# jy2k/Kubeflow-v2-distributed-pytorch

Measured on AMD Instinct MI355X. Metric: samples/sec (whole node) task.py DDP at 1/2/4/8 MI355X; scaling efficiency, higher is better.
Workload: dtype bf16; 1 GPU; model=resnet50, global_batch=256, image_size=224, batch_per_gpu=256, parallelism=dp1, impl=mipipe, optimizer=SGD(lr=0.1,momentum=0.9,wd=1e-4), hip_graph=True, deterministic=False, force_reduce=False, comm_dtype=fp32, native_reducer=False

## Files before the change

### csrc/bindings.cpp

```cpp
#include <torch/extension.h>

#include <unordered_map>

#include "bind/common.hpp"

using namespace mipipe_bind;

namespace {

void check_conv_buf_bytes(const mipipe::ConvShape& s, bool f32, const char* what) {
  if (f32) return;
  const int64_t lim = (1ll << 31) - (1ll << 24);
  TORCH_CHECK((int64_t)s.N * s.H * s.W * s.Ci * 2 < lim && (int64_t)s.N * s.Ho * s.Wo * s.Co * 2 < lim,
              "bf16 ", what, " tensors beyond 2 GiB are not supported");
}

mipipe::ConvShape make_conv_shape(int64_t N, int64_t H, int64_t W, int64_t Ci, int64_t Co, int KH,
                                  int KW, int stride, int pad, int stride_w, int pad_w, bool f32) {
  mipipe::ConvShape s;
  s.N = (int)N; s.H = (int)H; s.W = (int)W; s.Ci = (int)Ci;
  s.Co = (int)Co; s.KH = KH; s.KW = KW; s.stride = stride; s.pad = pad;
  s.stride_w = stride_w > 0 ? stride_w : 0;
  s.pad_w = pad_w >= 0 ? pad_w : -1;
  s.f32 = f32;
// ... 277 lines not shown
      mipipe::conv_fwd_infer(x.data_ptr(), w.data_ptr(), ys.data_ptr(), s, stream(), scp, shp, rp,
                             relu, c, wsp(ws));
    });
  }
  Tensor ws = split_ws(mipipe::conv_fwd_split_ws_elems(s, cfg), x);
  mipipe::conv_fwd_infer(x.data_ptr(), w.data_ptr(), y.data_ptr(), s, stream(), scp, shp, rp, relu,
                         cfg, wsp(ws));
  return y;
}

Tensor conv_dgrad(Tensor dy, Tensor w, std::vector<int64_t> x_shape, int stride, int pad,
                  optional<Tensor> addend, optional<Tensor> bn_y, optional<Tensor> bn_mean,
                  optional<Tensor> bn_invstd, optional<Tensor> bn_scale, optional<Tensor> bn_bias,
                  optional<Tensor> bn_rep, optional<Tensor> bn_z, int pad_w, int cfg,
                  optional<Tensor> bn_mask, optional<Tensor> bn_y2, optional<Tensor> bn_mean2,
                  optional<Tensor> bn_invstd2, optional<Tensor> wflip_pre) {
  check_act(dy, "dy");
  check_same(w, dy, "w");
  c10::DeviceGuard g(dy.device());
  TORCH_CHECK(x_shape.size() == 4, "x_shape must be [N,H,W,Ci]");
  const auto s = make_conv_shape(x_shape[0], x_shape[1], x_shape[2], x_shape[3], w.size(0),
                                 (int)w.size(1), (int)w.size(2), stride, pad, 0, pad_w, is_f32(dy));
  TORCH_CHECK(w.size(3) == s.Ci, "weight/input channel mismatch");
  const int pw = pad_w >= 0 ? pad_w : pad;
  TORCH_CHECK(dy.size(0) == s.N && dy.size(1) == s.Ho && dy.size(2) == s.Wo && dy.size(3) == s.Co,
              "dy shape does not match the convolution");
  TORCH_CHECK(s.Ci % 8 == 0 && s.Co % 8 == 0, "conv dgrad needs Ci, Co % 8 == 0");
  TORCH_CHECK(dy.numel() < (1ll << 31), "conv dgrad dy too large for 32-bit gather offsets");
  check_conv_buf_bytes(s, s.f32, "conv dgrad");
  TORCH_CHECK(s.pad < s.KH && pw < s.KW, "conv dgrad expects padding < kernel size");
  auto dx = torch::empty({s.N, s.H, s.W, s.Ci}, dy.options());
// ... 6 lines not shown
    if (wflip_pre.has_value() && mipipe::dgrad_preflip_ok(s)) {
      check_same(*wflip_pre, w, "wflip_pre");
      TORCH_CHECK(wflip_pre->numel() == w.numel() && wflip_pre->is_contiguous(),
                  "wflip_pre must match w's size");
      wfp = wflip_pre->data_ptr();
      preflipped = true;
    } else {
      wflip = torch::empty({(int64_t)s.Ci * s.KH * s.KW * s.Co}, w.options());
      wfp = wflip.data_ptr();
    }
  }
  mipipe::DgradFusion fz;
  bool any = false;
  if (addend.has_value()) {
    check_same(*addend, dy, "addend");
    TORCH_CHECK(addend->sizes() == dx.sizes(), "addend must match dx");
    fz.addend = addend->data_ptr();
    any = true;
  }
  if (bn_rep.has_value()) {
    TORCH_CHECK(bn_y.has_value() && bn_mean.has_value() && bn_invstd.has_value() &&
                bn_scale.has_value() && bn_bias.has_value(), "BN fusion needs y/mean/invstd/scale/bias");
    check_same(*bn_y, dy, "bn_y");
    TORCH_CHECK(bn_y->sizes() == dx.sizes(), "bn_y must match dx");
    check_vec(*bn_mean, s.Ci, "bn_mean");
    check_vec(*bn_invstd, s.Ci, "bn_invstd");
    check_vec(*bn_scale, s.Ci, "bn_scale");
    check_vec(*bn_bias, s.Ci, "bn_bias");
    check_f32(*bn_rep, "bn_rep");
    TORCH_CHECK(bn_rep->numel() == 3ll * mipipe::kStatReplicas * s.Ci, "bn_rep must be [3,R,Ci]");
    for (const Tensor* t : {&*bn_mean, &*bn_invstd, &*bn_scale, &*bn_bias})
      TORCH_CHECK(reinterpret_cast<uintptr_t>(t->data_ptr()) % 16 == 0,
                  "BN fusion vectors must be 16-byte aligned (the epilogue reads them as float4)");
// ... 1572 lines not shown
  m.attr("BN_ROW_ITERS") = mipipe::kBnRowIters;
  m.attr("DET_CHUNK_ROWS") = mipipe::kDetChunkRows;
  m.def("bn_bwd_reduce_blocks", [](int64_t M, int64_t C) {
    TORCH_CHECK(M >= 0 && C >= 8 && C % 8 == 0, "bn_bwd_reduce_blocks: M >= 0, C % 8 == 0");
    return mipipe::bn_bwd_reduce_blocks((long)M, (int)C);
  });
  m.def("bn_apply_u", []() { return mipipe::bn_apply_u(); });
  m.def("conv_dgrad", &conv_dgrad, py::arg("dy"), py::arg("w"), py::arg("x_shape"),
        py::arg("stride"), py::arg("pad"), py::arg("addend") = py::none(),
        py::arg("bn_y") = py::none(), py::arg("bn_mean") = py::none(),
        py::arg("bn_invstd") = py::none(), py::arg("bn_scale") = py::none(),
        py::arg("bn_bias") = py::none(), py::arg("bn_rep") = py::none(),
        py::arg("bn_z") = py::none(), py::arg("pad_w") = -1, py::arg("cfg") = -1,
        py::arg("bn_mask") = py::none(), py::arg("bn_y2") = py::none(),
        py::arg("bn_mean2") = py::none(), py::arg("bn_invstd2") = py::none(),
        py::arg("wflip_pre") = py::none());
  m.def("dgrad_preflip_ok", [](std::vector<int64_t> x_shape, std::vector<int64_t> w_shape,
                               int stride, int pad) {
    return mipipe::dgrad_preflip_ok(make_conv_shape(x_shape[0], x_shape[1], x_shape[2], x_shape[3],
                                                    w_shape[0], (int)w_shape[1], (int)w_shape[2],
                                                    stride, pad, 0, -1, false));
  });
  m.def("bn_bwd_collect", &bn_bwd_collect, py::arg("rep"), py::arg("C"),
        py::arg("dgamma") = py::none(), py::arg("dbeta") = py::none());
  m.def("conv_wgrad", &conv_wgrad, py::arg("dy"), py::arg("x"), py::arg("kh"), py::arg("kw"),
        py::arg("stride"), py::arg("pad"), py::arg("out") = py::none(), py::arg("stride_w") = 0,
        py::arg("pad_w") = -1, py::arg("cfg") = -1, py::arg("col_rep") = py::none(),
        py::arg("col_out") = py::none(), py::arg("col_dgamma") = py::none(),
        py::arg("col_dbeta") = py::none(), py::arg("col_two") = false,
        py::arg("col_dgamma2") = py::none(), py::arg("col_dbeta2") = py::none(),
        py::arg("in_scale") = py::none(), py::arg("in_bias") = py::none());
// ... 149 lines not shown
```

### csrc/kernels/conv_common.hpp

```cpp
#pragma once
#include "epilogue.hpp"
#include "gemm_pp.hpp"
#include "launchers.hpp"

namespace mipipe {
namespace gk {

static __device__ __attribute__((aligned(64))) uint4 g_conv_zero[8];

template <int BM_, int BN_, int NS_, int WM_, int WN_, bool PP_ = false>
struct Tile {
  static constexpr int BM = BM_, BN = BN_, NS = NS_, WM = WM_, WN = WN_;
  static constexpr int NW = WM * WN;
  static constexpr int THREADS = 64 * NW;
  static constexpr bool PP = PP_;
};

typedef Tile<128, 128, 2, 2, 2> T0;
typedef Tile<128, 128, 1, 2, 2> T1;
typedef Tile<128, 64, 2, 2, 2> T2;
typedef Tile<256, 128, 2, 4, 2> T3;
typedef Tile<256, 128, 3, 4, 2> T4;
typedef Tile<128, 256, 2, 2, 4> T5;
typedef Tile<256, 256, 2, 4, 2> T6;
// ... 109 lines not shown
  if (std::is_same<T, float>::value && f32_stages<C::BM, C::BN>() == 2) return 1;
  return C::NW == 8 ? (C::BM * C::BN <= 128 * 128 ? 2 : 1)
                    : ((C::NS == 1 && !std::is_same<T, float>::value) ? 3 : 2);
}

template <class T, class C, bool SPLIT>
constexpr int conv_fwd_lds_bytes() {
  return SPLIT && lds_bytes_f32out<T, C>() > lds_bytes_out<T, C>() ? lds_bytes_f32out<T, C>()
                                                                   : lds_bytes_out<T, C>();
}
template <class T, class C, bool BNIN>
constexpr int bnin_lds_bytes() {
  return BNIN ? main_lds_bytes<T, C>() + kBnInMaxK * 8 : 0;
}
template <class C, bool DENSE, bool ALIGNED, class T, bool DGRAD_EPI = false, bool SPLIT = false,
          bool BNIN = false>
__global__ __launch_bounds__(C::THREADS, (conv_occ<T, C>())) void conv_fwd_kernel(
    const T* __restrict__ x, const T* __restrict__ w, ConvGeom g, uint32_t M,
    uint32_t tilesN, EpiParams e) {
  constexpr int BM = C::BM, BN = C::BN;
  static_assert(!BNIN || (DENSE && !C::PP && !SPLIT && !DGRAD_EPI), "folded-BN forward variant");
  typedef typename std::conditional<
      BNIN, PolKCDenseBN<T>,
      typename std::conditional<DENSE, PolKCDense<T>, PolKCIm2col<ALIGNED, T>>::type>::type PA;
  constexpr int kLds = conv_fwd_lds_bytes<T, C, SPLIT>() > bnin_lds_bytes<T, C, BNIN>()
                           ? conv_fwd_lds_bytes<T, C, SPLIT>()
                           : bnin_lds_bytes<T, C, BNIN>();
  __shared__ __attribute__((aligned(16))) char smem[kLds];
  const int wave = __builtin_amdgcn_readfirstlane(threadIdx.x >> 6);
  const int lane = threadIdx.x & 63;
  uint32_t ntile = gridDim.x;
  if constexpr (!DGRAD_EPI) {
    if (e.fl_wt != nullptr) {
      if (blockIdx.x >= e.fl_tiles) {
        if (SPLIT && blockIdx.y != 0) return;
        flip_block<T, C::THREADS>(e, blockIdx.x - e.fl_tiles, smem);
// ... 23 lines not shown
    else a.init(x, g, M, origin, wave, lane, g_conv_zero);
    if constexpr (BNIN) a.tab = bn_tab;
  };
  auto ib = [&](auto& b, uint32_t origin) { b.init(w, K, e.N, K, origin, wave, lane, g_conv_zero); };
  f32x4 acc[BM / C::WM / 16][BN / C::WN / 16];
  run_main_loop<T, C, PA, PolKCDense<T>>(smem, ia, ib, m0, n0, kt0, kt1, acc, wave, lane);
  if constexpr (SPLIT) {
    EpiParams ws{};
    ws.C = e.split_ws;
    ws.ldc = e.N;
    ws.M = M;
    ws.N = e.N;
    ws.det_rows = 1;
    epilogue_f32<BM, BN, true, C::WM, C::WN, C::PP>(smem, acc, ws, m0, n0, wave, lane);
  } else {
    epilogue_out<BM, BN, DGRAD_EPI, T, C::WM, C::WN, false, C::PP>(smem, acc, e, m0, n0, 0, wave,
                                                                   lane);
  }
}

template <class T, class C>
constexpr int finish_lds_bytes() {
  constexpr int a = kEpiLdsBytes<C::BM, C::BN, T, C::WM>();
  constexpr int b = 16 * (C::THREADS + 8) * 4;
  return a > b ? a : b;
}
template <class C, class T, bool FUSE>
__global__ __launch_bounds__(C::THREADS) void conv_splitk_finish_kernel(
    const float* __restrict__ ws, int S, uint32_t tilesN, EpiParams e) {
  constexpr int BM = C::BM, BN = C::BN, WM = C::WM, WN = C::WN;
  constexpr int MT = BM / WM / 16, NT = BN / WN / 16;
  __shared__ __attribute__((aligned(16))) char smem[finish_lds_bytes<T, C>()];
  const int wave = __builtin_amdgcn_readfirstlane(threadIdx.x >> 6);
  const int lane = threadIdx.x & 63;
  const uint32_t tm = blockIdx.x / tilesN, tn = blockIdx.x % tilesN;
  const uint32_t m0 = tm * BM, n0 = tn * BN;
  const int wr = wave / WN, wc = wave % WN;
  typedef AccMap<BM, BN, WM, WN, false> Map;
  const uint32_t lr = lane & 15, lc = (lane >> 4) * 4;
  const long slice = (long)e.M * e.N;
  long off[MT][NT];
#pragma unroll
// ... 10 lines not shown
#pragma unroll
    for (int j = 0; j < NT; ++j) {
      const float4 v = *reinterpret_cast<const float4*>(ws + off[i][j]);
      acc[i][j] = f32x4{v.x, v.y, v.z, v.w};
    }
  for (int s = 1; s < S; ++s) {
    const float* wsl = ws + s * slice;
#pragma unroll
    for (int i = 0; i < MT; ++i)
#pragma unroll
      for (int j = 0; j < NT; ++j) {
        const float4 v = *reinterpret_cast<const float4*>(wsl + off[i][j]);
        acc[i][j] += f32x4{v.x, v.y, v.z, v.w};
      }
  }
  epilogue_out<BM, BN, FUSE, T, WM, WN, false, false>(smem, acc, e, m0, n0, 0, wave, lane);
}

template <class C, bool DENSE, bool ALIGNED, class T, bool TWO = false>
__global__ __launch_bounds__(C::THREADS, (conv_occ<T, C>())) void conv_dgrad_kernel(
    const T* __restrict__ dy, const T* __restrict__ w, int Ho, int Wo, int Co, int taps,
    FastDiv fCo, DgradClass cls, uint32_t M, uint32_t tilesN, EpiParams e) {
  constexpr int BM = C::BM, BN = C::BN;
  typedef typename std::conditional<DENSE, PolKCDense<T>, PolKCDgrad<ALIGNED, T>>::type PA;
  typedef typename std::conditional<DENSE, PolMCDense<T>, PolMCDgradW<ALIGNED, T>>::type PB;
  __shared__ __attribute__((aligned(16))) char smem[lds_bytes_out<T, C>()];
  const int wave = __builtin_amdgcn_readfirstlane(threadIdx.x >> 6);
  const int lane = threadIdx.x & 63;
  const uint32_t id = xcd_remap(blockIdx.x, gridDim.x);
  const uint32_t tm = id / tilesN, tn = id % tilesN;
  const uint32_t m0 = tm * BM, n0 = tn * BN;
  const uint32_t Ci = e.N;
  const uint32_t K = (uint32_t)(cls.ntaps * Co);
  const int nk = (int)((K + BK - 1) / BK);
  auto ia = [&](auto& a, uint32_t origin) {
    if constexpr (DENSE) a.init(dy, Co, M, K, origin, wave, lane, g_conv_zero);
    else a.init(dy, Ho, Wo, Co, fCo, cls, M, origin, wave, lane, g_conv_zero);
  };
  auto ib = [&](auto& b, uint32_t origin) {
    if constexpr (DENSE) b.init(w, Ci, Ci, K, origin, wave, lane, g_conv_zero);
    else b.init(w, (uint32_t)Co, (uint32_t)taps, Ci, fCo, cls, origin, wave, lane, g_conv_zero);
  };
  f32x4 acc[BM / C::WM / 16][BN / C::WN / 16];
  run_main_loop<T, C, PA, PB>(smem, ia, ib, m0, n0, 0, nk, acc, wave, lane);
  epilogue_out<BM, BN, true, T, C::WM, C::WN, TWO, C::PP>(smem, acc, e, m0, n0, 0, wave, lane);
}

template <class C, bool DENSE, class T, bool ATOMIC = true, bool BNIN = false>
__global__ __launch_bounds__(C::THREADS, (conv_occ<T, C>())) void conv_wgrad_kernel(
    const T* __restrict__ dy, const T* __restrict__ x, ConvGeom g, uint32_t tilesN,
    int kt_per_split, EpiParams e) {
  constexpr int BM = C::BM, BN = C::BN;
  static_assert(!BNIN || (DENSE && !C::PP), "folded-BN weight-grad variant");
  typedef typename std::conditional<
      BNIN, PolMCDenseBN<T>,
      typename std::conditional<DENSE, PolMCDense<T>, PolMCIm2colT<T>>::type>::type PB;
  __shared__ __attribute__((aligned(16))) char smem[lds_bytes_f32out<T, C>()];
  const int wave = __builtin_amdgcn_readfirstlane(threadIdx.x >> 6);
  const int lane = threadIdx.x & 63;
  const SplitPos pos = splitk_pos(e.xcd_splits);
// ... 81 lines not shown
```

### csrc/kernels/conv_dgrad.hip

```cpp
#include "conv_common.hpp"

namespace mipipe {
using namespace gk;

int default_dgrad_cfg(const ConvShape& s, long K_class) {
  const bool dense = is_dense(s);
  const bool ns1 = !s.f32 && (dense ? s.Co <= g_ns1_max_k
                                    : (s.Co % BK == 0 && K_class <= g_ns1_max_k_gather));
  if (s.Ci <= 64) return 2;
  return ns1 ? 1 : 0;
}

template <class F>
static void for_each_class(const ConvShape& s, F&& f) {
  const int S = s.stride;
  const int PW = s.pad_w >= 0 ? s.pad_w : s.pad;
  for (int ph = 0; ph < S; ++ph) {
    for (int pw = 0; pw < S; ++pw) {
      DgradClass c{};
      c.ph = ph; c.pw = pw;
      c.Hc = (s.H - ph + S - 1) / S;
      c.Wc = (s.W - pw + S - 1) / S;
      if (c.Hc <= 0 || c.Wc <= 0) continue;
      c.S = S; c.KW = s.KW;
// ... 134 lines not shown
      e.nt = ((g_nt_store >> 1) & 1) &&
             (long)s.N * s.H * s.W * s.Ci * (s.f32 ? 4 : 2) > g_nt_min_bytes;
      e.ntl = (g_nt_store >> 8) & 1;
      if (fz != nullptr) {
        e.addend = fz->addend;
        e.bnr_y = fz->bn_y;
        e.bnr_mean = fz->bn_mean; e.bnr_invstd = fz->bn_invstd;
        e.bnr_scale = fz->bn_scale; e.bnr_bias = fz->bn_bias; e.bnr_rep = fz->bn_rep; e.st_R = g_stat_rows;
        e.bnr_z = fz->bn_z;
        e.bnr_mask = fz->bn_mask;
        e.bnr_y2 = fz->bn_y2;
        e.bnr_mean2 = fz->bn_mean2;
        e.bnr_invstd2 = fz->bn_invstd2;
        e.det_rows = fz->det_rows;
        e.det_row0 = row0;
      }
      if (S > 1) {
        e.rm_s = S; e.rm_ph = c.ph; e.rm_pw = c.pw; e.rm_H = s.H; e.rm_W = s.W;
        e.rm_Hc = c.Hc; e.rm_Wc = c.Wc; e.rm_fHcWc = c.fHcWc; e.rm_fWc = c.fWc;
      }
      const int taps = s.KH * s.KW;
      const int cfg = resolve_dgrad_cfg(s, cfg_in, (long)c.ntaps * s.Co);
      if (wflip != nullptr && c.ntaps > 0 && e.bnr_y2 == nullptr) {
        T* wt = (T*)wflip + flip_off;
        flip_off += (long)s.Ci * c.ntaps * s.Co;
        if (!preflipped) weight_flip<T>(wp, wt, s, c, nkh, st);
        ConvShape s2 = s;
        s2.H = s.Ho; s2.W = s.Wo; s2.Ci = s.Co; s2.Co = s.Ci;
        s2.Ho = c.Hc; s2.Wo = c.Wc;
        s2.KH = nkh; s2.KW = c.nkw;
        s2.stride = 1; s2.stride_w = 0;
// ... 9 lines not shown
          const uint32_t tN = cdiv(s.Ci, C::BN), tiles = cdiv(M, C::BM) * tN;
          row0 += (int)cdiv(M, C::BM);
          const dim3 grid(tiles), block(C::THREADS);
          constexpr bool kSplitOk = !(C::BM == 256 && C::BN == 256 && !C::PP);
          if constexpr (kSplitOk) if (SK > 1) {
            EpiParams es = e;
            es.split_kt = kps;
            es.split_ws = split_ws;
            const dim3 g2d(tiles, SK);
            if (dense2)
              hipLaunchKernelGGL((conv_fwd_kernel<C, true, false, T, true, true>), g2d, block, 0, st, dyp, wt, g2, M, tN, es);
            else if (aligned && (s.f32 || nkh * c.nkw <= 32))
              hipLaunchKernelGGL((conv_fwd_kernel<C, false, true, T, true, true>), g2d, block, 0, st, dyp, wt, g2, M, tN, es);
            else
              hipLaunchKernelGGL((conv_fwd_kernel<C, false, false, T, true, true>), g2d, block, 0, st, dyp, wt, g2, M, tN, es);
            hipLaunchKernelGGL((conv_splitk_finish_kernel<C, T, true>), dim3(tiles), block, 0, st,
                               (const float*)split_ws, SK, tN, e);
            return;
          }
          if (dense2)
            hipLaunchKernelGGL((conv_fwd_kernel<C, true, false, T, true>), grid, block, 0, st, dyp, wt, g2, M, tN, e);
          else if (aligned && (s.f32 || nkh * c.nkw <= 32))
            hipLaunchKernelGGL((conv_fwd_kernel<C, false, true, T, true>), grid, block, 0, st, dyp, wt, g2, M, tN, e);
          else
            hipLaunchKernelGGL((conv_fwd_kernel<C, false, false, T, true>), grid, block, 0, st, dyp, wt, g2, M, tN, e);
        });
        return;
      }
      with_tile<T>(cfg, [&](auto tile) {
        typedef decltype(tile) C;
        const uint32_t tN = cdiv(s.Ci, C::BN), tiles = cdiv(M, C::BM) * tN;
        row0 += (int)cdiv(M, C::BM);
        const dim3 grid(tiles), block(C::THREADS);
        if (e.bnr_y2 != nullptr) {
          if constexpr (std::is_same<T, __bf16>::value)
            hipLaunchKernelGGL((conv_dgrad_kernel<C, true, false, T, true>), grid, block, 0, st, dyp, wp, s.Ho, s.Wo, s.Co, taps, fCo, c, M, tN, e);
        } else if (dense)
          hipLaunchKernelGGL((conv_dgrad_kernel<C, true, false, T>), grid, block, 0, st, dyp, wp, s.Ho, s.Wo, s.Co, taps, fCo, c, M, tN, e);
        else if (aligned && (s.f32 || c.ntaps <= 32))
          hipLaunchKernelGGL((conv_dgrad_kernel<C, false, true, T>), grid, block, 0, st, dyp, wp, s.Ho, s.Wo, s.Co, taps, fCo, c, M, tN, e);
        else
          hipLaunchKernelGGL((conv_dgrad_kernel<C, false, false, T>), grid, block, 0, st, dyp, wp, s.Ho, s.Wo, s.Co, taps, fCo, c, M, tN, e);
      });
  });
}

void conv_dgrad(const void* dy, const void* w, void* dx, const ConvShape& s, hipStream_t st,
                const DgradFusion* fz, int cfg, void* w_flip, bool preflipped, float* split_ws) {
  preflipped = preflipped && w_flip != nullptr && dgrad_preflip_ok(s);
  if (s.f32) conv_dgrad_t<float>(dy, w, dx, s, st, fz, cfg, w_flip, preflipped, split_ws);
  else conv_dgrad_t<__bf16>(dy, w, dx, s, st, fz, cfg, w_flip, preflipped, split_ws);
}

}
```

### csrc/kernels/epilogue.hpp

```cpp
#pragma once
#include "gemm_core.hpp"
#include "launchers.hpp"

namespace mipipe {
namespace gk {

struct EpiParams {
  void* C;
  long ldc;
  uint32_t M, N;
  const float* bias;
  int act;
  float* st_sum;
  float* st_sq;
  const float* st_shift;
  int st_R;
  int rm_s, rm_ph, rm_pw, rm_H, rm_W, rm_Hc, rm_Wc;
  FastDiv rm_fHcWc, rm_fWc;
  const void* addend;
  const void* bnr_y;
  const float *bnr_mean, *bnr_invstd, *bnr_scale, *bnr_bias;
  float* bnr_rep;
  const void* bnr_z;
  const void* bnr_y2;
// ... 6 lines not shown
  WsFinish fin;
  int xcd_splits;
  int nt, ntl;
  void* aux;
  const void* fl_w;
  void* fl_wt;
  int fl_Co, fl_KH, fl_KW, fl_Ci;
  uint32_t fl_tiles;
  FlipPlan fl;
  int split_kt;
  float* split_ws;
  const float* in_scale;
  const float* in_bias;
  const uint8_t* pf_ptr[2];
  uint32_t pf_lines[2];
};

template <int THREADS>
__device__ __forceinline__ uint32_t pf_issue(const EpiParams& e, uint32_t b, uint32_t nb) {
  uint32_t acc = 0;
  if (e.pf_lines[0] != 0) {
#pragma unroll
    for (int r = 0; r < 2; ++r) {
      const uint32_t per = (e.pf_lines[r] + nb - 1) / nb;
      const uint32_t l1 = min(e.pf_lines[r], (b + 1) * per);
      for (uint32_t l = b * per + threadIdx.x; l < l1; l += THREADS)
        acc += *reinterpret_cast<const uint32_t*>(e.pf_ptr[r] + ((size_t)l << 6));
    }
  }
  return acc;
// ... 159 lines not shown
  uint32_t rem = m - img * (uint32_t)(e.rm_Hc * e.rm_Wc);
  uint32_t i = fdiv(e.rm_fWc, rem);
  uint32_t j = rem - i * (uint32_t)e.rm_Wc;
  return ((long)img * e.rm_H + e.rm_ph + e.rm_s * (long)i) * e.rm_W + e.rm_pw + e.rm_s * (long)j;
}

template <int BN, class T = __bf16>
constexpr int kEpiPitch() { return BN * (int)sizeof(T) + 16; }
template <int BM, int BN, class T = __bf16>
constexpr int kStatsLdsOffset() { return ((BM * kEpiPitch<BN, T>()) + 255) / 256 * 256; }
template <int BM, int BN, class T = __bf16, int WM = 2>
constexpr int kEpiLdsBytes() { return kStatsLdsOffset<BM, BN, T>() + 2 * WM * BN * 4; }

__device__ __attribute__((aligned(64))) uint4 g_epi_zero[4];

template <int BM, int BN, bool FUSE, class T, int WM, int WN, bool TWO = false>
struct EpiOps {
  static constexpr int kThreads = 64 * WM * WN;
  static constexpr int CPR = BN / 8;
  static constexpr int ITER = BM * CPR / kThreads;
  static constexpr int PF = FUSE ? (ITER < 4 ? ITER : 4) : 1;
  Raw8<T> ad[PF], y[PF], z[PF], y2[TWO ? PF : 1];
  uint32_t mk[PF];
  const T *p_ad, *p_y, *p_z, *p_y2;
  const uint8_t* p_mk;
  bool h_ad, h_y, h_z, h_y2, h_mk;
  __device__ __forceinline__ void setup(const EpiParams& e) {
    const T* zt = reinterpret_cast<const T*>(g_epi_zero);
    const bool bnr = e.bnr_rep != nullptr;
    h_ad = e.addend != nullptr;
    h_y = bnr;
// ... 3 lines not shown
    p_ad = h_ad ? reinterpret_cast<const T*>(e.addend) : zt;
    p_y = h_y ? reinterpret_cast<const T*>(e.bnr_y) : zt;
    p_z = h_z ? reinterpret_cast<const T*>(e.bnr_z) : zt;
    p_y2 = h_y2 ? reinterpret_cast<const T*>(e.bnr_y2) : zt;
    p_mk = h_mk ? e.bnr_mask : reinterpret_cast<const uint8_t*>(g_epi_zero);
  }
  __device__ __forceinline__ void issue(const EpiParams& e, uint32_t m0, uint32_t n0, int it,
                                        int slot) {
    const uint32_t my_n = n0 + (threadIdx.x % CPR) * 8;
    const uint32_t ld_n = my_n < e.N ? my_n : 0;
    const uint32_t r = (threadIdx.x + it * kThreads) / CPR;
    const uint32_t m = min(m0 + r, e.M - 1);
    const long orow = out_row(e, m);
    const long off = orow * e.ldc + ld_n;
    const bool ntl = e.ntl != 0;
    ad[slot] = ld_raw8(p_ad + (h_ad ? off : 0), ntl);
    y[slot] = ld_raw8(p_y + (h_y ? off : 0), ntl);
    z[slot] = ld_raw8(p_z + (h_z ? off : 0), ntl);
    if constexpr (TWO) y2[slot] = ld_raw8(p_y2 + (h_y2 ? off : 0), ntl);
    mk[slot] = p_mk[h_mk ? off / 8 : 0];
  }
  __device__ __forceinline__ void prime(const EpiParams& e, uint32_t m0, uint32_t n0) {
    setup(e);
    if (FUSE && (e.addend != nullptr || e.bnr_rep != nullptr)) {
#pragma unroll
      for (int it = 0; it < PF; ++it) issue(e, m0, n0, it, it);
    }
  }
};

#ifndef MIPIPE_VALU_STATS
// ... 43 lines not shown
        if (e.det_rows > 0) {
          const long row = (long)(e.det_row0 + m0 / BM) * e.N + n;
          e.st_sum[row] = a;
          e.st_sq[row] = b;
        } else {
          const long row = (long)(blockIdx.x % e.st_R) * e.N + n;
          atomicAdd(e.st_sum + row, a);
          atomicAdd(e.st_sq + row, b);
        }
      }
    }
  }
}

template <int BM, int BN, bool FUSE = false, class T = __bf16, int WM = 2, int WN = 2,
          bool TWO = false, bool HALVES = false>
__device__ void epilogue_out(char* smem, f32x4 (&acc)[BM / WM / 16][BN / WN / 16],
                             const EpiParams& e, uint32_t m0, uint32_t n0, uint32_t prow_base,
                             int wave, int lane,
                             EpiOps<BM, BN, FUSE, T, WM, WN, TWO>* early = nullptr) {
  constexpr int MT = BM / WM / 16, NT = BN / WN / 16;
  constexpr int kThreads = 64 * WM * WN;
#ifdef MIPIPE_BNR_CENTERED
  constexpr bool kBnrUncentered = false;
#else
  constexpr bool kBnrUncentered = !std::is_same<T, float>::value;
#endif
  const int wr = wave / WN, wc = wave % WN;
  typedef AccMap<BM, BN, WM, WN, HALVES> Map;
  const uint32_t lr = lane & 15, lc = (lane >> 4) * 4;
  constexpr int CPR = BN / 8;
  constexpr int ITER = BM * CPR / kThreads;
  static_assert(kThreads % CPR == 0 && (BM * CPR) % kThreads == 0, "epilogue thread map");
  const bool bnr = FUSE && e.bnr_rep != nullptr;
  const bool has_add = FUSE && e.addend != nullptr;
  const bool zmask = bnr && e.bnr_z != nullptr && e.bnr_mask == nullptr;
  const bool bmask = bnr && e.bnr_mask != nullptr;
  const uint32_t my_cc = threadIdx.x % CPR, my_n = n0 + my_cc * 8;
  const uint32_t ld_n = my_n < e.N ? my_n : 0;
  typedef EpiOps<BM, BN, FUSE, T, WM, WN, TWO> Ops;
  constexpr int PF = Ops::PF;
  Ops local;
  Ops& ops = early != nullptr ? *early : local;
  (void)ld_n;
  float b_sc[8], b_bi[8], b_mu[8], b_is[8];
  if (bnr) {
    const bool okc = my_n < e.N;
    const uint32_t cn = okc ? my_n : 0;
    if (!bmask && !zmask) {
      ld_f32x8(e.bnr_scale + cn, b_sc);
      ld_f32x8(e.bnr_bias + cn, b_bi);
    } else {
#pragma unroll
      for (int q = 0; q < 8; ++q) b_sc[q] = b_bi[q] = 0.f;
    }
// ... 362 lines not shown
```

### csrc/kernels/launchers.hpp

```cpp
#pragma once
#include <hip/hip_runtime.h>
#include <stdint.h>

#include "plan.hpp"

namespace mipipe {

struct ConvShape {
  int N, H, W, Ci;
  int Co, KH, KW, stride, pad;
  int Ho, Wo;
  int stride_w = 0;
  int pad_w = -1;
  bool f32 = false;
};

constexpr int kStatReplicas = 16;
extern int g_stat_rows;
constexpr int kV8RowU = 4;
constexpr int kV8ApplyU = 2;
constexpr int kV8ReduceBlocks = 1024;
constexpr int kV8ApplyBlocks = 4096;
constexpr int kChanGridBlocks = 2048;
constexpr int kGridForBlocks = 8192;
// ... 55 lines not shown
struct FlipClass {
  int kh0, kw0, nkh, nkw;
  long off;
  uint32_t b0;
};
struct FlipPlan {
  FlipClass cls[4];
  int ncls = 0, S = 1;
  uint32_t nblk = 0;
};
void dgrad_flip_plan(const ConvShape& s, FlipPlan& p);
int dgrad_fwd_style_mode();
int conv_fwd_tiles_m(const ConvShape& s, int cfg);
struct DgradFusion {
  const void* addend = nullptr;
  const void* bn_y = nullptr;
  const float *bn_mean = nullptr, *bn_invstd = nullptr, *bn_scale = nullptr, *bn_bias = nullptr;
  float* bn_rep = nullptr;
  const void* bn_z = nullptr;
  const uint8_t* bn_mask = nullptr;
  const void* bn_y2 = nullptr;
  const float *bn_mean2 = nullptr, *bn_invstd2 = nullptr;
  int det_rows = 0;
};
void conv_dgrad(const void* dy, const void* w, void* dx, const ConvShape& s, hipStream_t st,
                const DgradFusion* fz = nullptr, int cfg = -1, void* w_flip = nullptr,
                bool preflipped = false, float* split_ws = nullptr);
bool conv_dgrad_fwd_style(const ConvShape& s, bool dense_too);
int conv_dgrad_tiles_m(const ConvShape& s, int cfg);
struct BnCollect {
// ... 270 lines not shown
```

### kubeflow-v2-distributed-pytorch_amd/ops/functional.py

```python
from __future__ import annotations

import math
import os
import weakref
from dataclasses import dataclass
from typing import Optional, Tuple

import torch
from torch.autograd import Function

from . import kernels as K
from . import prefetch as _prefetch

Tensor = torch.Tensor


_RELU_BITMASK = os.environ.get("MIPIPE_RELU_BITMASK", "1") != "0"

_SIDE_WGRAD = os.environ.get("MIPIPE_SIDE_WGRAD", "0") == "1"
_SIDE_STREAMS = {}
_SIDE_JOIN_PENDING = set()


def _side_stream(t: Tensor):
# ... 33 lines not shown
        return fs, fs.padded_view(fs.flat_grad, p)
    return fs, g


def _wgrad_map_into_grad(wmap, dw, weight):
    acc = getattr(wmap, "accumulate_into", None)
    tgt = _direct_grad_target(weight) if acc is not None else None
    if tgt is not None and acc(dw, tgt[1]):
        tgt[0].grad_ready(weight)
        return None
    return wmap(dw).to(weight.dtype)


class ResidualSlot:

    __slots__ = ("pending", "consumed")

    def __init__(self):
        self.pending = None
        self.consumed = False

    def produce(self, g):
        if g is None or self.consumed:
            return g
        self.pending = g if self.pending is None else self.pending + g
        return None

    def take(self):
        self.consumed = True
        p, self.pending = self.pending, None
        return p


class BiasGradSlot:

    __slots__ = ("bias", "done")

    def __init__(self):
        self.bias = None
        self.done = False


class BNActToken:

    __slots__ = ("bn", "st", "y", "_z", "mask", "pre_reduced", "collected", "y2", "st2", "bn2",
                 "rep")
# ... 5 lines not shown
    @z.setter
    def z(self, t):
        self._z = None if t is None else weakref.ref(t)

    def __init__(self, bn, st, y, z=None):
        self.bn, self.st, self.y, self.z = bn, st, y, z
        self.mask = None
        self.pre_reduced = False
        self.collected = None
        self.y2 = self.st2 = self.bn2 = None
        self.rep = None


_TAP_CROP = os.environ.get("MIPIPE_TAP_CROP", "1") != "0"
_CONV_FLATTEN = os.environ.get("MIPIPE_CONV_FLATTEN", "1") != "0"


def tap_crop(x_shape, w_shape, stride, pad):
    if not (_TAP_CROP and isinstance(stride, int) and isinstance(pad, int)):
        return None
    _, H, W, _ = x_shape
    _, KH, KW, _ = w_shape
    Ho, Wo = (H + 2 * pad - KH) // stride + 1, (W + 2 * pad - KW) // stride + 1

    def span(L, Lo, K):
        used = [k for k in range(K) if any(0 <= o * stride - pad + k < L for o in range(Lo))]
        return (used[0], used[-1] + 1) if used else (0, K)
    (h0, h1), (w0, w1) = span(H, Ho, KH), span(W, Wo, KW)
    if (h0, h1, w0, w1) == (0, KH, 0, KW) or pad - h0 != pad - w0:
        return None
# ... 50 lines not shown
        return y, psum, psumsq

    @staticmethod
    def backward(ctx, dy, _g1, _g2):
        x, w_c = ctx.saved_tensors
        if dy is None:
            return (None,) * 11
        in_bn = ctx.in_bn
        stride, pad, kh, kw, ci = ctx.conf
        dy = dy.contiguous()
        dx = dw = None
        bnr = tok = None
        if ctx.needs_input_grad[0]:
            if not isinstance(stride, int):
                raise NotImplementedError("dgrad of a non-square-stride conv")
            addend = ctx.res_take.take() if ctx.res_take is not None else None
            bnr = None
            tok = ctx.prev if ctx.flat is None else None
            if ctx.flat is not None and addend is not None:
                addend = addend.reshape(x.shape)
            two = tok is not None and tok.y2 is not None
            two_ok = (not two or (kh == 1 and kw == 1 and stride == 1 and pad == 0
                                  and dy.dtype == torch.bfloat16 and ctx.needs_input_grad[1]
                                  and tok.st2.batch_stats))
            if (tok is not None and K.use_native(dy) and tok.st.batch_stats and two_ok
                    and (tok.z is None or addend is not None)):
                rep = bn_workspace(tok.bn, "bwd", dy.device)
                tok.rep = rep
                if rep is not None:
                    st = tok.st
                    bnr = (tok.y, st.mean, st.invstd, st.scale, st.bias, rep)
                    if tok.z is not None:
                        bnr = bnr + (tok.mask if tok.mask is not None else tok.z,)
            bnr2 = (tok.y2, tok.st2.mean, tok.st2.invstd) if bnr is not None and two else None
            dx = K.conv_dgrad(dy, w_c, x.shape, stride, pad, addend=addend, bnr=bnr, bnr2=bnr2,
                              wflip=ctx.wflip)
            if bnr is not None:
                tok.pre_reduced = True
            if ctx.flat is not None:
                dx = dx.reshape(ctx.flat)
            if ctx.res_give is not None:
                dx = ctx.res_give.produce(dx)
        if ctx.needs_input_grad[1]:
            weight = ctx.weight
            collect = None
            cin = x.shape[-1] if ctx.flat is None else ctx.flat[-1]
            tgt = (_direct_grad_target(weight)
                   if cin == ci and ctx.wmap is None and K.use_native(dy) else None)
            side = None
            if (_SIDE_WGRAD and tgt is not None and dy.is_cuda and not tgt[0]._ready_listeners
                    and not (bnr is not None and tok.y2 is not None) and ctx.crop is None):
                side = _side_stream(dy)
            if bnr is not None and side is None:
                two = tok.y2 is not None
                bn = tok.bn
                out2 = torch.empty(3 if two else 2, bn.num_features, device=dy.device,
                                   dtype=torch.float32)
# ... 644 lines not shown
        dy2 = dy.reshape(-1, dy.shape[-1]).contiguous()
        tb = None
        if ctx.has_bias and ctx.needs_input_grad[3] and K.use_native(dy2):
            tb = _direct_grad_target(ctx.bias, dy2.shape[1])
        bias_done = ctx.bias_slot is not None and ctx.bias_slot.done
        if ctx.act == "gelu":
            if tb is not None and K.gelu_bwd_colsum_ok(dy2):
                dy2 = K.gelu_bwd_colsum(dy2, aux, tb[1])
                bias_done = True
            else:
                dy2 = K.gelu_bwd(dy2, aux)
        elif ctx.act == "relu":
            dy2 = (dy2.float() * (aux > 0)).to(dy2.dtype)
        dx = dw = db = None
        if ctx.needs_input_grad[0]:
            add = ctx.res_take.take() if ctx.res_take is not None else None
            if add is not None:
                add = add.reshape(-1, add.shape[-1]).to(dy2.dtype).contiguous()
            pf = _prefetch.before_weight_gemm(w_c, [x2] if ctx.needs_input_grad[1] else None)
            dx = K.gemm(dy2, w_c, False, False, None, "none", dy2.dtype,
                        addend=add, prefetch=pf).reshape(ctx.shp)
        gdt = torch.float64 if dy2.dtype == torch.float64 else torch.float32
        if ctx.needs_input_grad[1]:
            tgt = _direct_grad_target(ctx.weight, w_c.shape[0]) if K.use_native(dy2) else None
            sink = getattr(ctx.weight, "_mipipe_sparse_sink", None)
            ready_now = sink is not None or not getattr(ctx.weight, "_mipipe_tied_later", False)
            if tgt is not None:
                fs, g = tgt
                K.gemm(dy2, x2, True, False, None, "none", torch.float32,
                       g.reshape(w_c.shape[0], -1), 1.0)
                if ready_now:
# ... 203 lines not shown

    @staticmethod
    def forward(ctx, x, weight, w_c, bias, res_give):
        y = K.dwconv7_fwd(x, w_c, None if bias is None else bias.detach())
        ctx.save_for_backward(x, w_c)
        ctx.weight, ctx.bias, ctx.res_give = weight, bias, res_give
        return y

    @staticmethod
    def backward(ctx, dy):
        x, w_c = ctx.saved_tensors
        weight, bias = ctx.weight, ctx.bias
        dy = dy.contiguous()
        dx = dw = db = None
        if ctx.needs_input_grad[0]:
            add = ctx.res_give.take() if ctx.res_give is not None else None
            if add is not None:
                add = add.reshape(dy.shape).to(dy.dtype)
            dx = K.dwconv7_dgrad(dy, w_c, add)
        need_w = ctx.needs_input_grad[1]
        need_b = bias is not None and ctx.needs_input_grad[3]
        if need_w or need_b:
            native = K.use_native(dy)
            tw = _direct_grad_target(weight) if native and need_w else None
            tb = _direct_grad_target(bias) if native and need_b else None
            g_w, g_b = K.dwconv7_wgrad(dy, x, None if tw is None else tw[1].reshape(-1),
                                       None if tb is None else tb[1])
            if tw is not None:
                tw[0].grad_ready(weight)
            elif need_w:
                dw = g_w.reshape(weight.shape).to(weight.dtype)
# ... 181 lines not shown
```

### kubeflow-v2-distributed-pytorch_amd/ops/kernels.py

```python
from __future__ import annotations

import os
from typing import NamedTuple, Optional

import torch

from . import _ref
from ._ref import _f
from ._native import native, native_available

__all__ = ["conv_fwd", "conv_fwd_infer", "bn_fold_affine", "conv_dgrad", "conv_wgrad", "bn_finalize", "bn_act_fwd",
           "bn_act_bwd_reduce", "bn_act_bwd_apply", "maxpool_fwd", "maxpool_bwd",
           "avgpool_fwd", "avgpool_bwd", "pool_bn_fwd", "pool_bn_bwd", "pool_bn_supported", "stem_fused_supported", "stem_fwd_stats",
           "stem_fwd_pool", "stem_bwd", "gemm", "cross_entropy_fwd_bwd", "cross_entropy_mixed_fwd_bwd",
           "batch_mix", "top1_correct", "eval_stats", "sgd_step",
           "adamw_step", "ema_update", "ema_swap", "ema_buffers_update", "ema_buffers_swap",
           "layernorm_fwd", "layernorm_bwd", "patchify", "tokens_assemble_fwd", "tokens_assemble_bwd", "attention_fwd", "attention_bwd", "dropout_fwd", "colsum", "bn_bwd_collect", "stem_pack",
           "embedding_bwd", "gelu_fwd", "gelu_bwd", "nchw_to_nhwc", "record_decode", "record_decode_rrc",
           "record_augment", "batch_erase_",
           "use_native",
           "gconv_fwd", "gconv_dgrad", "gconv_wgrad", "chan_stats", "affine_act",
           "bn_generic_bwd_reduce", "bn_generic_bwd_apply", "avgpool2d_fwd", "avgpool2d_bwd",
           "dwconv7_fwd", "dwconv7_dgrad", "dwconv7_wgrad", "drop_path_keep",
           "scale_residual_fwd", "scale_residual_bwd"]
# ... 47 lines not shown
                               residual, relu)


def bn_fold_affine(weight, bias, running_mean, running_var, eps, conv_bias=None):
    if use_native(weight):
        return native().bn_fold_affine(weight, bias, running_mean, running_var, eps, conv_bias)
    return _ref.bn_fold_affine(weight, bias, running_mean, running_var, eps, conv_bias)


def dgrad_preflip_ok(x_shape, w_shape, stride, pad) -> bool:
    if not (isinstance(stride, int) and isinstance(pad, int)) or not native_available():
        return False
    return bool(native().dgrad_preflip_ok(list(x_shape), list(w_shape), stride, pad))


def conv_dgrad(dy, w, x_shape, stride, pad, addend=None, bnr=None, bnr2=None, wflip=None):
    if use_native(dy):
        ph, pw = _pads(pad)
        if bnr is None:
            return native().conv_dgrad(dy, w, list(x_shape), stride, ph, addend, pad_w=pw,
                                       wflip_pre=wflip)
        y, mean, invstd, scale, bias, rep = bnr[:6]
        z = bnr[6] if len(bnr) > 6 else None
        mask = None
        if z is not None and z.dtype == torch.uint8:
            z, mask = None, z
        y2, mean2, invstd2 = bnr2 if bnr2 is not None else (None, None, None)
        return native().conv_dgrad(dy, w, list(x_shape), stride, ph, addend, y, mean, invstd,
                                   scale, bias, rep, z, pw, bn_mask=mask, bn_y2=y2,
                                   bn_mean2=mean2, bn_invstd2=invstd2, wflip_pre=wflip)
    if bnr is not None:
        raise RuntimeError("BN-reduce dgrad fusion is a native-kernel path")
    dx = _ref.conv_dgrad(dy, w, x_shape, stride, pad if isinstance(pad, int) else tuple(pad))
    return dx if addend is None else (dx + addend).to(dx.dtype)


def bn_bwd_collect(rep, C, acc=None):
    a = acc if acc is not None else (None, None)
    return native().bn_bwd_collect(rep, C, *a)


def conv_wgrad(dy, x, kh, kw, stride, pad, out=None, collect=None, in_bn=None):
    sh, sw = (stride, 0) if isinstance(stride, int) else (stride[0], stride[1])
    if use_native(dy):
        ph, pw = _pads(pad)
        c = tuple(collect) if collect is not None else (None, None, None, None)
        if len(c) == 4:
# ... 625 lines not shown
```

Measured before the change: 13460 samples/s.

## Fuse strided downsample-shortcut gradient into dense 1x1 dgrad epilogue as compact addend

For strided 1x1 pad-0 downsample convs, the data-grad is now computed as a stride-1 dense dgrad on the compact grid rather than the full-resolution strided dgrad. The compact result is handed to the residual slot and consumed by the sibling 1x1 dgrad epilogue, which scatters it through a strided-addend index calculation. This avoids writing and reading a mostly-zero full-size gradient tensor and the strided dgrad kernel. In exchange it adds extra kernel template variants, fast-division index math in the epilogue, and a Python fallback that expands to the full shape when the fused path cannot apply.

```diff
diff --git a/csrc/bindings.cpp b/csrc/bindings.cpp
--- a/csrc/bindings.cpp
+++ b/csrc/bindings.cpp
@@ -315,7 +315,7 @@
                   optional<Tensor> bn_invstd, optional<Tensor> bn_scale, optional<Tensor> bn_bias,
                   optional<Tensor> bn_rep, optional<Tensor> bn_z, int pad_w, int cfg,
                   optional<Tensor> bn_mask, optional<Tensor> bn_y2, optional<Tensor> bn_mean2,
-                  optional<Tensor> bn_invstd2, optional<Tensor> wflip_pre) {
+                  optional<Tensor> bn_invstd2, optional<Tensor> wflip_pre, int addend_stride) {
   check_act(dy, "dy");
   check_same(w, dy, "w");
   c10::DeviceGuard g(dy.device());
@@ -352,9 +352,27 @@
   bool any = false;
   if (addend.has_value()) {
     check_same(*addend, dy, "addend");
-    TORCH_CHECK(addend->sizes() == dx.sizes(), "addend must match dx");
+    TORCH_CHECK(addend_stride >= 1, "addend_stride must be >= 1");
+    if (addend_stride > 1) {
+      const int64_t Hc = (s.H + addend_stride - 1) / addend_stride;
+      const int64_t Wc = (s.W + addend_stride - 1) / addend_stride;
+      TORCH_CHECK(mipipe::conv_is_dense(s),
+                  "a strided addend needs a 1x1 / stride-1 / pad-0 data-grad");
+      TORCH_CHECK(addend->numel() == (int64_t)s.N * Hc * Wc * s.Ci,
+                  "strided addend must hold N*ceil(H/s)*ceil(W/s)*Ci = ", s.N * Hc * Wc * s.Ci,
+                  " elements, got ", addend->numel());
+      TORCH_CHECK(reinterpret_cast<uintptr_t>(addend->data_ptr()) % 16 == 0,
+                  "strided addend must be 16-byte aligned");
+      fz.ad_s = addend_stride;
+      fz.ad_Hc = (int)Hc;
+      fz.ad_Wc = (int)Wc;
+    } else {
+      TORCH_CHECK(addend->sizes() == dx.sizes(), "addend must match dx");
+    }
     fz.addend = addend->data_ptr();
     any = true;
+  } else {
+    TORCH_CHECK(addend_stride == 1, "addend_stride without an addend");
   }
   if (bn_rep.has_value()) {
     TORCH_CHECK(bn_y.has_value() && bn_mean.has_value() && bn_invstd.has_value() &&
@@ -1957,7 +1975,7 @@
         py::arg("bn_z") = py::none(), py::arg("pad_w") = -1, py::arg("cfg") = -1,
         py::arg("bn_mask") = py::none(), py::arg("bn_y2") = py::none(),
         py::arg("bn_mean2") = py::none(), py::arg("bn_invstd2") = py::none(),
-        py::arg("wflip_pre") = py::none());
+        py::arg("wflip_pre") = py::none(), py::arg("addend_stride") = 1);
   m.def("dgrad_preflip_ok", [](std::vector<int64_t> x_shape, std::vector<int64_t> w_shape,
                                int stride, int pad) {
     return mipipe::dgrad_preflip_ok(make_conv_shape(x_shape[0], x_shape[1], x_shape[2], x_shape[3],
diff --git a/csrc/kernels/conv_common.hpp b/csrc/kernels/conv_common.hpp
--- a/csrc/kernels/conv_common.hpp
+++ b/csrc/kernels/conv_common.hpp
@@ -147,12 +147,13 @@
   return BNIN ? main_lds_bytes<T, C>() + kBnInMaxK * 8 : 0;
 }
 template <class C, bool DENSE, bool ALIGNED, class T, bool DGRAD_EPI = false, bool SPLIT = false,
-          bool BNIN = false>
+          bool BNIN = false, bool ADS = false>
 __global__ __launch_bounds__(C::THREADS, (conv_occ<T, C>())) void conv_fwd_kernel(
     const T* __restrict__ x, const T* __restrict__ w, ConvGeom g, uint32_t M,
     uint32_t tilesN, EpiParams e) {
   constexpr int BM = C::BM, BN = C::BN;
   static_assert(!BNIN || (DENSE && !C::PP && !SPLIT && !DGRAD_EPI), "folded-BN forward variant");
+  static_assert(!ADS || (DENSE && DGRAD_EPI), "strided addend: dense data-grads only");
   typedef typename std::conditional<
       BNIN, PolKCDenseBN<T>,
       typename std::conditional<DENSE, PolKCDense<T>, PolKCIm2col<ALIGNED, T>>::type>::type PA;
@@ -206,8 +207,8 @@
     ws.det_rows = 1;
     epilogue_f32<BM, BN, true, C::WM, C::WN, C::PP>(smem, acc, ws, m0, n0, wave, lane);
   } else {
-    epilogue_out<BM, BN, DGRAD_EPI, T, C::WM, C::WN, false, C::PP>(smem, acc, e, m0, n0, 0, wave,
-                                                                   lane);
+    epilogue_out<BM, BN, DGRAD_EPI, T, C::WM, C::WN, false, C::PP, ADS>(smem, acc, e, m0, n0, 0,
+                                                                        wave, lane);
   }
 }
 
@@ -217,7 +218,7 @@
   constexpr int b = 16 * (C::THREADS + 8) * 4;
   return a > b ? a : b;
 }
-template <class C, class T, bool FUSE>
+template <class C, class T, bool FUSE, bool ADS = false>
 __global__ __launch_bounds__(C::THREADS) void conv_splitk_finish_kernel(
     const float* __restrict__ ws, int S, uint32_t tilesN, EpiParams e) {
   constexpr int BM = C::BM, BN = C::BN, WM = C::WM, WN = C::WN;
@@ -258,10 +259,10 @@
         acc[i][j] += f32x4{v.x, v.y, v.z, v.w};
       }
   }
-  epilogue_out<BM, BN, FUSE, T, WM, WN, false, false>(smem, acc, e, m0, n0, 0, wave, lane);
-}
-
-template <class C, bool DENSE, bool ALIGNED, class T, bool TWO = false>
+  epilogue_out<BM, BN, FUSE, T, WM, WN, false, false, ADS>(smem, acc, e, m0, n0, 0, wave, lane);
+}
+
+template <class C, bool DENSE, bool ALIGNED, class T, bool TWO = false, bool ADS = false>
 __global__ __launch_bounds__(C::THREADS, (conv_occ<T, C>())) void conv_dgrad_kernel(
     const T* __restrict__ dy, const T* __restrict__ w, int Ho, int Wo, int Co, int taps,
     FastDiv fCo, DgradClass cls, uint32_t M, uint32_t tilesN, EpiParams e) {
@@ -287,7 +288,8 @@
   };
   f32x4 acc[BM / C::WM / 16][BN / C::WN / 16];
   run_main_loop<T, C, PA, PB>(smem, ia, ib, m0, n0, 0, nk, acc, wave, lane);
-  epilogue_out<BM, BN, true, T, C::WM, C::WN, TWO, C::PP>(smem, acc, e, m0, n0, 0, wave, lane);
+  static_assert(!ADS || DENSE, "strided addend: dense data-grads only");
+  epilogue_out<BM, BN, true, T, C::WM, C::WN, TWO, C::PP, ADS>(smem, acc, e, m0, n0, 0, wave, lane);
 }
 
 template <class C, bool DENSE, class T, bool ATOMIC = true, bool BNIN = false>
diff --git a/csrc/kernels/conv_dgrad.hip b/csrc/kernels/conv_dgrad.hip
--- a/csrc/kernels/conv_dgrad.hip
+++ b/csrc/kernels/conv_dgrad.hip
@@ -1,3 +1,5 @@
+#include <stdexcept>
+
 #include "conv_common.hpp"
 
 namespace mipipe {
@@ -172,7 +174,14 @@
         e.bnr_invstd2 = fz->bn_invstd2;
         e.det_rows = fz->det_rows;
         e.det_row0 = row0;
+        if (fz->ad_s > 1) {
+          e.ad_s = fz->ad_s; e.ad_Hc = fz->ad_Hc; e.ad_Wc = fz->ad_Wc;
+          e.ad_fHW = FastDiv((uint32_t)(s.H * s.W));
+          e.ad_fW = FastDiv((uint32_t)s.W);
+          e.ad_fS = FastDiv((uint32_t)fz->ad_s);
+        }
       }
+      const bool ads = e.ad_s > 1;
       if (S > 1) {
         e.rm_s = S; e.rm_ph = c.ph; e.rm_pw = c.pw; e.rm_H = s.H; e.rm_W = s.W;
         e.rm_Hc = c.Hc; e.rm_Wc = c.Wc; e.rm_fHcWc = c.fHcWc; e.rm_fWc = c.fWc;
@@ -212,11 +221,17 @@
               hipLaunchKernelGGL((conv_fwd_kernel<C, false, true, T, true, true>), g2d, block, 0, st, dyp, wt, g2, M, tN, es);
             else
               hipLaunchKernelGGL((conv_fwd_kernel<C, false, false, T, true, true>), g2d, block, 0, st, dyp, wt, g2, M, tN, es);
-            hipLaunchKernelGGL((conv_splitk_finish_kernel<C, T, true>), dim3(tiles), block, 0, st,
-                               (const float*)split_ws, SK, tN, e);
+            if (ads)
+              hipLaunchKernelGGL((conv_splitk_finish_kernel<C, T, true, true>), dim3(tiles), block, 0, st,
+                                 (const float*)split_ws, SK, tN, e);
+            else
+              hipLaunchKernelGGL((conv_splitk_finish_kernel<C, T, true>), dim3(tiles), block, 0, st,
+                                 (const float*)split_ws, SK, tN, e);
             return;
           }
-          if (dense2)
+          if (dense2 && ads)
+            hipLaunchKernelGGL((conv_fwd_kernel<C, true, false, T, true, false, false, true>), grid, block, 0, st, dyp, wt, g2, M, tN, e);
+          else if (dense2)
             hipLaunchKernelGGL((conv_fwd_kernel<C, true, false, T, true>), grid, block, 0, st, dyp, wt, g2, M, tN, e);
           else if (aligned && (s.f32 || nkh * c.nkw <= 32))
             hipLaunchKernelGGL((conv_fwd_kernel<C, false, true, T, true>), grid, block, 0, st, dyp, wt, g2, M, tN, e);
@@ -231,9 +246,15 @@
         row0 += (int)cdiv(M, C::BM);
         const dim3 grid(tiles), block(C::THREADS);
         if (e.bnr_y2 != nullptr) {
-          if constexpr (std::is_same<T, __bf16>::value)
-            hipLaunchKernelGGL((conv_dgrad_kernel<C, true, false, T, true>), grid, block, 0, st, dyp, wp, s.Ho, s.Wo, s.Co, taps, fCo, c, M, tN, e);
-        } else if (dense)
+          if constexpr (std::is_same<T, __bf16>::value) {
+            if (ads)
+              hipLaunchKernelGGL((conv_dgrad_kernel<C, true, false, T, true, true>), grid, block, 0, st, dyp, wp, s.Ho, s.Wo, s.Co, taps, fCo, c, M, tN, e);
+            else
+              hipLaunchKernelGGL((conv_dgrad_kernel<C, true, false, T, true>), grid, block, 0, st, dyp, wp, s.Ho, s.Wo, s.Co, taps, fCo, c, M, tN, e);
+          }
+        } else if (dense && ads)
+          hipLaunchKernelGGL((conv_dgrad_kernel<C, true, false, T, false, true>), grid, block, 0, st, dyp, wp, s.Ho, s.Wo, s.Co, taps, fCo, c, M, tN, e);
+        else if (dense)
           hipLaunchKernelGGL((conv_dgrad_kernel<C, true, false, T>), grid, block, 0, st, dyp, wp, s.Ho, s.Wo, s.Co, taps, fCo, c, M, tN, e);
         else if (aligned && (s.f32 || c.ntaps <= 32))
           hipLaunchKernelGGL((conv_dgrad_kernel<C, false, true, T>), grid, block, 0, st, dyp, wp, s.Ho, s.Wo, s.Co, taps, fCo, c, M, tN, e);
@@ -246,6 +267,8 @@
 void conv_dgrad(const void* dy, const void* w, void* dx, const ConvShape& s, hipStream_t st,
                 const DgradFusion* fz, int cfg, void* w_flip, bool preflipped, float* split_ws) {
   preflipped = preflipped && w_flip != nullptr && dgrad_preflip_ok(s);
+  if (fz != nullptr && fz->ad_s > 1 && (!is_dense(s) || fz->addend == nullptr))
+    throw std::invalid_argument("conv_dgrad: a strided addend needs a dense 1x1 stride-1 data-grad");
   if (s.f32) conv_dgrad_t<float>(dy, w, dx, s, st, fz, cfg, w_flip, preflipped, split_ws);
   else conv_dgrad_t<__bf16>(dy, w, dx, s, st, fz, cfg, w_flip, preflipped, split_ws);
 }
diff --git a/csrc/kernels/epilogue.hpp b/csrc/kernels/epilogue.hpp
--- a/csrc/kernels/epilogue.hpp
+++ b/csrc/kernels/epilogue.hpp
@@ -44,6 +44,8 @@
   const float* in_bias;
   const uint8_t* pf_ptr[2];
   uint32_t pf_lines[2];
+  int ad_s, ad_Hc, ad_Wc;
+  FastDiv ad_fHW, ad_fW, ad_fS;
 };
 
 template <int THREADS>
@@ -233,7 +235,7 @@
 
 __device__ __attribute__((aligned(64))) uint4 g_epi_zero[4];
 
-template <int BM, int BN, bool FUSE, class T, int WM, int WN, bool TWO = false>
+template <int BM, int BN, bool FUSE, class T, int WM, int WN, bool TWO = false, bool ADS = false>
 struct EpiOps {
   static constexpr int kThreads = 64 * WM * WN;
   static constexpr int CPR = BN / 8;
@@ -267,7 +269,17 @@
     const long orow = out_row(e, m);
     const long off = orow * e.ldc + ld_n;
     const bool ntl = e.ntl != 0;
-    ad[slot] = ld_raw8(p_ad + (h_ad ? off : 0), ntl);
+    if constexpr (ADS) {
+      const uint32_t img = fdiv(e.ad_fHW, m);
+      const uint32_t rem = m - img * e.ad_fHW.d;
+      const uint32_t h = fdiv(e.ad_fW, rem), w = rem - h * e.ad_fW.d;
+      const uint32_t hc = fdiv(e.ad_fS, h), wc = fdiv(e.ad_fS, w);
+      const bool on = h_ad & (hc * e.ad_fS.d == h) & (wc * e.ad_fS.d == w);
+      const long aoff = (((long)img * e.ad_Hc + hc) * e.ad_Wc + wc) * e.ldc + ld_n;
+      ad[slot] = ld_raw8(on ? p_ad + aoff : reinterpret_cast<const T*>(g_epi_zero), ntl);
+    } else {
+      ad[slot] = ld_raw8(p_ad + (h_ad ? off : 0), ntl);
+    }
     y[slot] = ld_raw8(p_y + (h_y ? off : 0), ntl);
     z[slot] = ld_raw8(p_z + (h_z ? off : 0), ntl);
     if constexpr (TWO) y2[slot] = ld_raw8(p_y2 + (h_y2 ? off : 0), ntl);
@@ -341,11 +353,11 @@
 }
 
 template <int BM, int BN, bool FUSE = false, class T = __bf16, int WM = 2, int WN = 2,
-          bool TWO = false, bool HALVES = false>
+          bool TWO = false, bool HALVES = false, bool ADS = false>
 __device__ void epilogue_out(char* smem, f32x4 (&acc)[BM / WM / 16][BN / WN / 16],
                              const EpiParams& e, uint32_t m0, uint32_t n0, uint32_t prow_base,
                              int wave, int lane,
-                             EpiOps<BM, BN, FUSE, T, WM, WN, TWO>* early = nullptr) {
+                             EpiOps<BM, BN, FUSE, T, WM, WN, TWO, ADS>* early = nullptr) {
   constexpr int MT = BM / WM / 16, NT = BN / WN / 16;
   constexpr int kThreads = 64 * WM * WN;
 #ifdef MIPIPE_BNR_CENTERED
@@ -365,7 +377,7 @@
   const bool bmask = bnr && e.bnr_mask != nullptr;
   const uint32_t my_cc = threadIdx.x % CPR, my_n = n0 + my_cc * 8;
   const uint32_t ld_n = my_n < e.N ? my_n : 0;
-  typedef EpiOps<BM, BN, FUSE, T, WM, WN, TWO> Ops;
+  typedef EpiOps<BM, BN, FUSE, T, WM, WN, TWO, ADS> Ops;
   constexpr int PF = Ops::PF;
   Ops local;
   Ops& ops = early != nullptr ? *early : local;
diff --git a/csrc/kernels/launchers.hpp b/csrc/kernels/launchers.hpp
--- a/csrc/kernels/launchers.hpp
+++ b/csrc/kernels/launchers.hpp
@@ -93,6 +93,7 @@
 int conv_fwd_tiles_m(const ConvShape& s, int cfg);
 struct DgradFusion {
   const void* addend = nullptr;
+  int ad_s = 0, ad_Hc = 0, ad_Wc = 0;
   const void* bn_y = nullptr;
   const float *bn_mean = nullptr, *bn_invstd = nullptr, *bn_scale = nullptr, *bn_bias = nullptr;
   float* bn_rep = nullptr;
diff --git a/kubeflow-v2-distributed-pytorch_amd/ops/functional.py b/kubeflow-v2-distributed-pytorch_amd/ops/functional.py
--- a/kubeflow-v2-distributed-pytorch_amd/ops/functional.py
+++ b/kubeflow-v2-distributed-pytorch_amd/ops/functional.py
@@ -71,22 +71,45 @@
 
 class ResidualSlot:
 
-    __slots__ = ("pending", "consumed")
+    __slots__ = ("pending", "consumed", "stride", "full_shape")
 
     def __init__(self):
         self.pending = None
         self.consumed = False
-
-    def produce(self, g):
-        if g is None or self.consumed:
+        self.stride = 1
+        self.full_shape = None
+
+    @staticmethod
+    def expand(g, stride, full_shape):
+        if stride == 1:
             return g
-        self.pending = g if self.pending is None else self.pending + g
+        full = g.new_zeros(tuple(full_shape))
+        full[:, ::stride, ::stride, :] = g
+        return full
+
+    def produce(self, g, stride=1, full_shape=None):
+        if g is None:
+            return g
+        if self.consumed:
+            return self.expand(g, stride, full_shape)
+        if self.pending is None:
+            self.pending, self.stride = g, stride
+            self.full_shape = tuple(full_shape) if stride != 1 else None
+        elif stride == self.stride and (stride == 1 or tuple(full_shape) == self.full_shape):
+            self.pending = self.pending + g
+        else:
+            self.pending = (self.expand(self.pending, self.stride, self.full_shape)
+                            + self.expand(g, stride, full_shape))
+            self.stride, self.full_shape = 1, None
         return None
 
-    def take(self):
+    def take(self, strided=False):
         self.consumed = True
-        p, self.pending = self.pending, None
-        return p
+        p, s, shape = self.pending, self.stride, self.full_shape
+        self.pending, self.stride, self.full_shape = None, 1, None
+        if p is not None and s != 1 and not strided:
+            p, s = self.expand(p, s, shape), 1
+        return p, s
 
 
 class BiasGradSlot:
@@ -122,6 +145,7 @@
 
 _TAP_CROP = os.environ.get("MIPIPE_TAP_CROP", "1") != "0"
 _CONV_FLATTEN = os.environ.get("MIPIPE_CONV_FLATTEN", "1") != "0"
+_DS_COMPACT = os.environ.get("MIPIPE_DS_COMPACT", "1") != "0"
 
 
 def tap_crop(x_shape, w_shape, stride, pad):
@@ -202,7 +226,14 @@
         if ctx.needs_input_grad[0]:
             if not isinstance(stride, int):
                 raise NotImplementedError("dgrad of a non-square-stride conv")
-            addend = ctx.res_take.take() if ctx.res_take is not None else None
+            addend, ad_s = None, 1
+            if ctx.res_take is not None:
+                addend, ad_s = ctx.res_take.take(
+                    strided=(_DS_COMPACT and ctx.flat is None and kh == 1 and kw == 1
+                             and stride == 1 and pad == 0 and K.use_native(dy)))
+            compact = (_DS_COMPACT and ctx.res_give is not None and not ctx.res_give.consumed
+                       and ctx.flat is None and ctx.res_take is None and ctx.prev is None
+                       and kh == 1 and kw == 1 and pad == 0 and stride > 1)
             bnr = None
             tok = ctx.prev if ctx.flat is None else None
             if ctx.flat is not None and addend is not None:
@@ -221,14 +252,19 @@
                     if tok.z is not None:
                         bnr = bnr + (tok.mask if tok.mask is not None else tok.z,)
             bnr2 = (tok.y2, tok.st2.mean, tok.st2.invstd) if bnr is not None and two else None
-            dx = K.conv_dgrad(dy, w_c, x.shape, stride, pad, addend=addend, bnr=bnr, bnr2=bnr2,
-                              wflip=ctx.wflip)
-            if bnr is not None:
-                tok.pre_reduced = True
-            if ctx.flat is not None:
-                dx = dx.reshape(ctx.flat)
-            if ctx.res_give is not None:
-                dx = ctx.res_give.produce(dx)
+            if compact:
+                n, h, w_ = x.shape[0], dy.shape[1], dy.shape[2]
+                dx = K.conv_dgrad(dy, w_c, (n, h, w_, x.shape[3]), 1, 0)
+                dx = ctx.res_give.produce(dx, stride, tuple(x.shape))
+            else:
+                dx = K.conv_dgrad(dy, w_c, x.shape, stride, pad, addend=addend, bnr=bnr,
+                                  bnr2=bnr2, wflip=ctx.wflip, addend_stride=ad_s)
+                if bnr is not None:
+                    tok.pre_reduced = True
+                if ctx.flat is not None:
+                    dx = dx.reshape(ctx.flat)
+                if ctx.res_give is not None:
+                    dx = ctx.res_give.produce(dx)
         if ctx.needs_input_grad[1]:
             weight = ctx.weight
             collect = None
@@ -903,7 +939,7 @@
             dy2 = (dy2.float() * (aux > 0)).to(dy2.dtype)
         dx = dw = db = None
         if ctx.needs_input_grad[0]:
-            add = ctx.res_take.take() if ctx.res_take is not None else None
+            add = ctx.res_take.take()[0] if ctx.res_take is not None else None
             if add is not None:
                 add = add.reshape(-1, add.shape[-1]).to(dy2.dtype).contiguous()
             pf = _prefetch.before_weight_gemm(w_c, [x2] if ctx.needs_input_grad[1] else None)
@@ -1137,7 +1173,7 @@
         dy = dy.contiguous()
         dx = dw = db = None
         if ctx.needs_input_grad[0]:
-            add = ctx.res_give.take() if ctx.res_give is not None else None
+            add = ctx.res_give.take()[0] if ctx.res_give is not None else None
             if add is not None:
                 add = add.reshape(dy.shape).to(dy.dtype)
             dx = K.dwconv7_dgrad(dy, w_c, add)
diff --git a/kubeflow-v2-distributed-pytorch_amd/ops/kernels.py b/kubeflow-v2-distributed-pytorch_amd/ops/kernels.py
--- a/kubeflow-v2-distributed-pytorch_amd/ops/kernels.py
+++ b/kubeflow-v2-distributed-pytorch_amd/ops/kernels.py
@@ -85,12 +85,13 @@
     return bool(native().dgrad_preflip_ok(list(x_shape), list(w_shape), stride, pad))
 
 
-def conv_dgrad(dy, w, x_shape, stride, pad, addend=None, bnr=None, bnr2=None, wflip=None):
+def conv_dgrad(dy, w, x_shape, stride, pad, addend=None, bnr=None, bnr2=None, wflip=None,
+               addend_stride=1):
     if use_native(dy):
         ph, pw = _pads(pad)
         if bnr is None:
             return native().conv_dgrad(dy, w, list(x_shape), stride, ph, addend, pad_w=pw,
-                                       wflip_pre=wflip)
+                                       wflip_pre=wflip, addend_stride=addend_stride)
         y, mean, invstd, scale, bias, rep = bnr[:6]
         z = bnr[6] if len(bnr) > 6 else None
         mask = None
@@ -99,9 +100,12 @@
         y2, mean2, invstd2 = bnr2 if bnr2 is not None else (None, None, None)
         return native().conv_dgrad(dy, w, list(x_shape), stride, ph, addend, y, mean, invstd,
                                    scale, bias, rep, z, pw, bn_mask=mask, bn_y2=y2,
-                                   bn_mean2=mean2, bn_invstd2=invstd2, wflip_pre=wflip)
+                                   bn_mean2=mean2, bn_invstd2=invstd2, wflip_pre=wflip,
+                                   addend_stride=addend_stride)
     if bnr is not None:
         raise RuntimeError("BN-reduce dgrad fusion is a native-kernel path")
+    if addend_stride != 1:
+        raise RuntimeError("a strided addend is a native-kernel path")
     dx = _ref.conv_dgrad(dy, w, x_shape, stride, pad if isinstance(pad, int) else tuple(pad))
     return dx if addend is None else (dx + addend).to(dx.dtype)
 
```

Measured after the change: 13530 samples/s, median of 6. No clear change (+0.5%).
